# dvl-tum/e-osvos

Measured on AMD Instinct MI355X. Metric: finetune_iters_per_sec, higher is better.
Workload: dtype f32 (f16x3 split); 1 GPU; e-OSVOS-50 fine-tune iteration (BASELINE configs[1]): DeepLabV3+-ResNet50, batch 3, 480x854, BCE, per-neuron-lr SGD; one (sequence, object) per rank; batch=3, height=480, width=854, parallelism=replicas x1

## Files before the change

### e-osvos_amd/csrc/conv_kernels.hip

```cpp
#include "kernels.h"

#include <stdlib.h>
#include <string.h>

#include <vector>

namespace eosvos {

typedef float f32x16 __attribute__((ext_vector_type(16)));

#define EOSVOS_BK 32
#define EOSVOS_EB 4
#define EOSVOS_EB128 EOSVOS_EB
#define EOSVOS_OCC 2
#define MFMA32(a, b, c) __builtin_amdgcn_mfma_f32_32x32x2f32((a), (b), (c), 0, 0, 0)

__device__ __forceinline__ int xcd_remap(int bid, int nwg) {
  const int q = nwg >> 3, r = nwg & 7, xcd = bid & 7;
  return (xcd < r ? xcd * (q + 1) : r * (q + 1) + (xcd - r) * q) + (bid >> 3);
}

__device__ __forceinline__ float4 ldg4(const float* p) { return *reinterpret_cast<const float4*>(p); }
__device__ __forceinline__ float4 bufld4(__amdgpu_buffer_rsrc_t r, unsigned byte_off) {
  auto v = __builtin_amdgcn_raw_buffer_load_b128(r, byte_off, 0, 0);
// ... 764 lines not shown
    const int ks_total = p.tprefix ? p.tprefix[tile + 1] - p.tprefix[tile] : ksteps;
    unsigned long long tappack = 0x876543210ULL;
    if (!MULTI && p.tprefix) {
      const int mask = p.tmask[tile];
      tappack = 0;
      int nv = 0;
      for (int t2 = 0; t2 < T; ++t2)
        if ((mask >> t2) & 1) { tappack |= (unsigned long long)t2 << (4 * nv); ++nv; }
    }
    const int m0 = (tile / nt) * BM, n0 = (tile % nt) * BN;

    int a_sy0[APASS], a_sx0[APASS], a_img[APASS];
#pragma unroll
    for (int i = 0; i < APASS; ++i) {
      int m = m0 + a_r + i * 32;
      if (m < p.M) {
        if (p.par) m = conv_par_pixel(p.B, p.Ho, p.Wo, m);
        const int hw = p.Ho * p.Wo;
        const int b = m / hw, rem = m - b * hw;
        const int oy = rem / p.Wo, ox = rem - oy * p.Wo;
        a_sy0[i] = oy * p.mul + p.off0;
        a_sx0[i] = ox * p.mul + p.off0;
        a_img[i] = b * p.Hi * p.Wi;
      } else {
        a_sy0[i] = -(1 << 28);
        a_sx0[i] = 0;
        a_img[i] = 0;
      }
    }
    float4 ra[APASS], rb[BPASS];
    constexpr unsigned OOB = 0x80000000u;
    int a_off[APASS];
    int b_off[BPASS];
    const int wplane = p.plane_rows ? (m0 / p.plane_rows) * (int)p.w_plane : 0;
#pragma unroll
    for (int i = 0; i < BPASS; ++i) {
      if (KMAJOR) {
        const int n = n0 + b_n4 * 4;
        b_off[i] = n < p.N ? wplane + (b_kq * RPT + i) * T * p.wK + n : -1;
      } else {
        const int n = n0 + b_r + i * 32;
        b_off[i] = n < p.N ? wplane + n * T * p.wK + b_c4 * 4 : -1;
      }
    }
    int cur_tap = -1;
    int m_wrow = 0, m_ksoff = 0;
    auto load_tiles = [&](int ks) {
      const int vt = ks / chunks;
      const int c0 = (ks - vt * chunks) * BK;
      const int tap = MULTI ? vt : (p.tprefix ? (int)((tappack >> (4 * vt)) & 15) : vt);
      if (tap != cur_tap) {
        cur_tap = tap;
        int dy, dx, xoff = 0;
        if (MULTI) {
          const int id = __builtin_amdgcn_readfirstlane((int)p.taplist[(size_t)tile * 32 + vt]);
          const ConvTap d = p.taps[id];
          dy = d.dy; dx = d.dx; xoff = d.xoff; m_wrow = d.wrow; m_ksoff = d.ksoff; seg_ld = d.seg;
          if (NP == 2) { sa = pick4(seg_sa, seg_ld); sb = pick4(seg_sb, seg_ld); }
#pragma unroll
          for (int i = 0; i < BPASS; ++i) {
            const int n = n0 + b_n4 * 4;
            b_off[i] = n < p.N ? d.wbase + (b_kq * RPT + i) * d.wrow + n : -1;
          }
        } else {
          const int ky = tap / p.KW, kx = tap - ky * p.KW;
          dy = ky * p.kstep; dx = kx * p.kstep;
        }
#pragma unroll
        for (int i = 0; i < APASS; ++i) {
          const int sy = a_sy0[i] + dy, sx = a_sx0[i] + dx;
          bool ok = sy >= 0 && sx >= 0 && ((sy | sx) & (up - 1)) == 0;
          const int iy = sy >> p.upshift, ix = sx >> p.upshift;
          ok = ok && iy < p.Hi && ix < p.Wi;
          a_off[i] = ok ? (a_img[i] + iy * p.Wi + ix) * p.ldx + a_c4 * 4 + xoff : -1;
        }
      }
      const bool cok = (c0 + a_c4 * 4) < p.Kc;
      float4 ks4 = make_float4(1.f, 1.f, 1.f, 1.f);
      if (KMAJOR && p.kscale && cok) ks4 = ldg4(p.kscale + (MULTI ? m_ksoff : 0) + c0 + a_c4 * 4);
#pragma unroll
      for (int i = 0; i < APASS; ++i) {
        const unsigned off = (cok && a_off[i] >= 0) ? (unsigned)(a_off[i] + c0) * 4u : OOB;
        float4 v = bufld4(rx, off);
        if (KMAJOR) { v.x *= ks4.x; v.y *= ks4.y; v.z *= ks4.z; v.w *= ks4.w; }
        ra[i] = v;
      }
#pragma unroll
      for (int i = 0; i < BPASS; ++i) {
        unsigned off;
        if (MULTI) {
          const int k = c0 + b_kq * RPT + i;
          off = (b_off[i] >= 0 && k < p.Kc) ? (unsigned)(b_off[i] + c0 * m_wrow) * 4u : OOB;
        } else if (KMAJOR) {
          const int k = c0 + b_kq * RPT + i;
          off = (b_off[i] >= 0 && k < p.Kc) ? (unsigned)(b_off[i] + (c0 * T + tap) * p.wK) * 4u : OOB;
        } else {
          const int k = c0 + b_c4 * 4;
          off = (b_off[i] >= 0 && k < p.Kc) ? (unsigned)(b_off[i] + tap * p.wK + c0) * 4u : OOB;
        }
        rb[i] = bufld4(rw, off);
      }
    };
    auto store_tiles = [&]() {
#pragma unroll
      for (int i = 0; i < APASS; ++i) {
        uint2 pc[NP];
        xs_split4<NP>(ra[i].x, ra[i].y, ra[i].z, ra[i].w, sa, pc);
#pragma unroll
        for (int q = 0; q < NP; ++q) *reinterpret_cast<uint2*>(As + (q * BM + a_r + i * 32) * X6_ROWB + a_c4 * 8) = pc[q];
      }
      if (!KMAJOR) {
#pragma unroll
        for (int i = 0; i < BPASS; ++i) {
          uint2 pc[NP];
          xs_split4<NP>(rb[i].x, rb[i].y, rb[i].z, rb[i].w, sb, pc);
#pragma unroll
          for (int q = 0; q < NP; ++q) *reinterpret_cast<uint2*>(Bs + (q * BN + b_r + i * 32) * X6_ROWB + b_c4 * 8) = pc[q];
        }
      } else if (RPT == 4) {
#pragma unroll
        for (int j = 0; j < 4; ++j) {
          uint2 pc[NP];
          xs_split4<NP>(f4c(rb[0], j), f4c(rb[1], j), f4c(rb[RPT == 4 ? 2 : 0], j), f4c(rb[RPT == 4 ? 3 : 0], j), sb, pc);
#pragma unroll
          for (int q = 0; q < NP; ++q) *reinterpret_cast<uint2*>(Bs + (q * BN + j * NQ + b_n4) * X6_ROWB + b_kq * 8) = pc[q];
        }
      } else {
#pragma unroll
        for (int j = 0; j < 4; ++j) {
          unsigned pc[NP];
          xs_split2<NP>(f4c(rb[0], j), f4c(rb[1], j), sb, pc);
#pragma unroll
          for (int q = 0; q < NP; ++q) *reinterpret_cast<unsigned*>(Bs + (q * BN + j * NQ + b_n4) * X6_ROWB + b_kq * 4) = pc[q];
        }
      }
    };

    constexpr int TM = 4;
    f32x4 acc[TM][TN];
#pragma unroll
    for (int i = 0; i < TM; ++i)
#pragma unroll
      for (int j = 0; j < TN; ++j)
#pragma unroll
        for (int e = 0; e < 4; ++e) acc[i][j][e] = 0.f;

    load_tiles(ks_begin);
    scales_late();
    __syncthreads();
    store_tiles();
    __syncthreads();
    if (MULTI) seg_acc = seg_ld;

    for (int ks = ks_begin; ks < ks_end; ++ks) {
      const bool more = (ks + 1) < ks_end;
      if (more) load_tiles(ks + 1);
      __builtin_amdgcn_s_setprio(1);
      x6_mma_step<TM, TN, ((BN == 128 && NP == 3) ? 2 : TM), NP>(As, Bs, BM, BN, wm * 64, wn * (BN / 2), fr, fq, acc);
      __builtin_amdgcn_s_setprio(0);
      __syncthreads();
      if (more) store_tiles();
      if (MULTI && NP == 2 && more && seg_ld != seg_acc) {
        const float f = pick4(seg_inv, seg_acc) / pick4(seg_inv, seg_ld);
#pragma unroll
        for (int i = 0; i < TM; ++i)
#pragma unroll
          for (int j = 0; j < TN; ++j)
#pragma unroll
            for (int e = 0; e < 4; ++e) acc[i][j][e] *= f;
        seg_acc = seg_ld;
      }
      __syncthreads();
    }
    if (MULTI && NP == 2) inv_ab = pick4(seg_inv, seg_acc);

    float* Cs = reinterpret_cast<float*>(smem);
    const bool full = p.splitk == 0 && ks_begin == 0 && ks_end == ks_total;
    constexpr int CF4 = BN / 4, CROWS = 256 / CF4;
    const int c_c4 = tid % CF4, c_r = tid / CF4;
    const int n = n0 + c_c4 * 4;
    float4 sc = make_float4(1.f, 1.f, 1.f, 1.f), bi = make_float4(0.f, 0.f, 0.f, 0.f);
    if (full && n < p.N) {
      if (p.scale) sc = ldg4(p.scale + n);
      if (p.bias) bi = ldg4(p.bias + n);
    }
    const bool use_mask8 = p.mask8 && n >= p.mask_c0;
    const bool write_m8 = p.mask8_out && p.relu;
    const float y2s = (NP == 2 && p.y2) ? *p.y2_sc : 0.f;
    {
#pragma unroll
      for (int tm = 0; tm < TM; ++tm)
#pragma unroll
        for (int tn = 0; tn < TN; ++tn) {
          const int Rb = wn * (BN / 2) + tn * 16 + fr;
          const int ncol = KMAJOR ? x6_row_chan(Rb, BN) : Rb;
#pragma unroll
          for (int e = 0; e < 4; ++e) Cs[(wm * 64 + tm * 16 + 4 * fq + e) * LDC + ncol] = NP == 2 ? acc[tm][tn][e] * inv_ab : acc[tm][tn][e];
        }
      __syncthreads();
      if (full) {
        if (n < p.N) {
          constexpr int NIT = BM / CROWS, EB = BN == 128 ? EOSVOS_EB128 : EOSVOS_EB;
          const float* const adp = p.res ? p.res : (p.accum ? p.y : nullptr);
          const int adld = p.res ? p.ldres : p.ldy;
          const bool both = p.res && p.accum;
#pragma unroll
          for (int it0 = 0; it0 < NIT; it0 += EB) {
            size_t md[EB];
            bool ok[EB];
            float4 ad[EB];
            unsigned mk8[EB];
#pragma unroll
            for (int j = 0; j < EB; ++j) {
              const int m = m0 + c_r + (it0 + j) * CROWS;
              ok[j] = m < p.M;
              md[j] = dst_pixel(p, ok[j] ? m : p.M - 1);
            }
            if (adp) {
#pragma unroll
              for (int j = 0; j < EB; ++j) ad[j] = ldg4(adp + md[j] * adld + n);
            }
            if (use_mask8) {
#pragma unroll
              for (int j = 0; j < EB; ++j) mk8[j] = p.mask8[md[j] * p.ldm8 + (n >> 2)];
            }
#pragma unroll
            for (int j = 0; j < EB; ++j) {
              float4 v = *reinterpret_cast<const float4*>(Cs + (c_r + (it0 + j) * CROWS) * LDC + c_c4 * 4);
              if (p.scale) { v.x *= sc.x; v.y *= sc.y; v.z *= sc.z; v.w *= sc.w; }
              if (p.bias) { v.x += bi.x; v.y += bi.y; v.z += bi.z; v.w += bi.w; }
              if (adp) { v.x += ad[j].x; v.y += ad[j].y; v.z += ad[j].z; v.w += ad[j].w; }
              if (both) { const float4 a2 = ldg4(p.y + md[j] * p.ldy + n); v.x += a2.x; v.y += a2.y; v.z += a2.z; v.w += a2.w; }
              if (p.relu) { v.x = fmaxf(v.x, 0.f); v.y = fmaxf(v.y, 0.f); v.z = fmaxf(v.z, 0.f); v.w = fmaxf(v.w, 0.f); }
              if (use_mask8) relu_mask8(v, mk8[j]);
              if (ok[j]) {
                *reinterpret_cast<float4*>(p.y + md[j] * p.ldy + n) = v;
                if (write_m8) p.mask8_out[md[j] * p.ldm8_out + (n >> 2)] = relu_bits(v);
                if (NP == 2 && p.y2) pair_store4(p.y2, md[j], p.ldy, n, v, y2s);
                if (NP == 2) ymax = amax_f4(ymax, v);
              }
            }
          }
        }
      } else {
        float* slab = p.ws + ((size_t)bid * 2 + (u == u_begin ? 0 : 1)) * (BM * BN);
#pragma unroll 4
        for (int lr = c_r; lr < BM; lr += CROWS)
          *reinterpret_cast<float4*>(slab + lr * BN + c_c4 * 4) = *reinterpret_cast<const float4*>(Cs + lr * LDC + c_c4 * 4);
      }
    }
    if (!dp) u += ks_end - ks_begin;
  }
  if (NP == 2 && p.amax_y) amax_block_commit(ymax, p.amax_y);
}

template <int BN, bool KMAJOR>
__global__ __launch_bounds__(256, 2) void conv_x6_kernel(const ConvArgs p) {
  __shared__ __attribute__((aligned(16))) unsigned char smem[conv_xs_smem<BN, 3>()];
  conv_xs_body<BN, KMAJOR, 3>(p, smem);
}
#define EOSVOS_H3_OCC64 2
template <int BN, bool KMAJOR>
__global__ __launch_bounds__(256, BN == 64 ? EOSVOS_H3_OCC64 : 2) void conv_h3_kernel(const ConvArgs p) {
  __shared__ __attribute__((aligned(16))) unsigned char smem[conv_xs_smem<BN, 2>()];
  conv_xs_body<BN, KMAJOR, 2>(p, smem);
}
__global__ __launch_bounds__(256, 2) void conv_h3_multi_kernel(const ConvArgs p) {
  __shared__ __attribute__((aligned(16))) unsigned char smem[conv_xs_smem<128, 2>()];
  conv_xs_body<128, true, 2, true>(p, smem);
}
__global__ __launch_bounds__(256, 2) void conv_x6_multi_kernel(const ConvArgs p) {
  __shared__ __attribute__((aligned(16))) unsigned char smem[conv_xs_smem<128, 3>()];
  conv_xs_body<128, true, 3, true>(p, smem);
}

__device__ __forceinline__ void amax_block_commit8(unsigned m, unsigned* slot) {
  __shared__ unsigned wmax8[8];
#pragma unroll
  for (int o = 32; o > 0; o >>= 1) {
    const unsigned t = (unsigned)__shfl_xor((int)m, o);
    m = m > t ? m : t;
  }
  if ((threadIdx.x & 63) == 0) wmax8[threadIdx.x >> 6] = m;
  __syncthreads();
  if (threadIdx.x == 0) {
    unsigned q = 0;
#pragma unroll
    for (int i = 0; i < 8; ++i) q = q > wmax8[i] ? q : wmax8[i];
    if (q) atomicMax(slot + (size_t)((blockIdx.x + blockIdx.y) & (AMAX_SUB - 1)) * AMAX_ROW, q);
  }
}
__device__ __forceinline__ void s1_split8(const float4& lo, const float4& hi, float s, uint4& h0, uint4& h1) {
  unsigned a[4], b[4];
  h3_split_pair(lo.x, lo.y, s, a[0], b[0]);
  h3_split_pair(lo.z, lo.w, s, a[1], b[1]);
  h3_split_pair(hi.x, hi.y, s, a[2], b[2]);
  h3_split_pair(hi.z, hi.w, s, a[3], b[3]);
  h0 = make_uint4(a[0], a[1], a[2], a[3]);
  h1 = make_uint4(b[0], b[1], b[2], b[3]);
}
constexpr int frag_pitch(int row_bytes) { return row_bytes % 64 == 32 ? row_bytes : row_bytes + (96 - row_bytes % 64) % 64; }
#define EOSVOS_STREAM3X3_D 6
#define EOSVOS_STREAM_OCC 1
template <int K, int NC>
__global__ __launch_bounds__(512, (K <= 128 ? EOSVOS_STREAM_OCC : 1)) void conv1x1_stream_kernel(const ConvArgs p) {
  constexpr int WAVES = 8;
  constexpr int KS = (K + 31) / 32;
  constexpr int PITCH = frag_pitch(K * 2);
  constexpr int NF = NC / 16;
  constexpr int FHM = (K >= 256 || EOSVOS_STREAM_OCC > 1) ? 4 : 8;
  constexpr int FH = NF < FHM ? NF : FHM;
  constexpr bool KOUT = K >= 304;
  constexpr bool KTAIL = (K % 32) != 0;
  extern __shared__ __attribute__((aligned(16))) unsigned char s1_smem[];
  const int tid = threadIdx.x, lane = tid & 63, wave = tid >> 6;
  int n0 = blockIdx.y * NC;
  long rbase = 0, rend = p.M;
  int sbeg = blockIdx.x * WAVES + wave, sstride = gridDim.x * WAVES;
  const float* wsrc = p.w;
  if (p.plane_rows) {
    const int ranges = p.N / NC, chunks = p.row_chunks;
    const int i = blockIdx.x, xcd = i & 7, j = i >> 3;
    const int g = (j / ranges) * 8 + xcd;
    if (g >= p.nplanes * chunks) return;
    const int plane = g / chunks, chunk = g % chunks;
    const long per = (((long)p.plane_rows + chunks - 1) / chunks + 15) / 16 * 16;
    n0 = (j % ranges) * NC;
    rbase = (long)plane * p.plane_rows + chunk * per;
    rend = rbase + per;
    if (rend > (long)(plane + 1) * p.plane_rows) rend = (long)(plane + 1) * p.plane_rows;
    sbeg = wave; sstride = WAVES;
    wsrc = p.w + (size_t)plane * p.w_plane;
  }
  float* const s_sc = reinterpret_cast<float*>(s1_smem + 2 * NC * PITCH);
  float* const s_bi = s_sc + NC;
  float* const s_ks = s_bi + NC;
  static_assert(NC <= WAVES * 64 && K <= WAVES * 64, "one factor per thread");
  const float f_sc = (p.scale && tid < NC) ? p.scale[n0 + tid] : 1.f;
  const float f_bi = (p.bias && tid < NC) ? p.bias[n0 + tid] : 0.f;
  const float f_ks = (p.kscale && tid < K) ? p.kscale[tid] : 1.f;
  const unsigned ax = amax_issue(p.amax_x), aks = amax_issue(p.kmajor ? p.amax_ks : nullptr), aw = amax_issue(p.amax_w);
  float sx = 1.f, sw = 1.f, inv = 1.f;
  auto scales = [&]() {
    if (tid < NC) { s_sc[tid] = f_sc; s_bi[tid] = f_bi; }
    if (tid < KS * 32) s_ks[tid] = f_ks;
    float ix, iw;
    sx = h3_scale_bits(ax, p.kmajor && p.amax_ks, aks, ix);
    sw = h3_scale_bits(aw, false, 0u, iw);
    inv = ix * iw;
  };
  {
    constexpr int GR = NC * (K / 8), IT = (GR + WAVES * 64 - 1) / (WAVES * 64);
    if (!p.kmajor) {
      float4 raw[IT][2];
#pragma unroll
      for (int it = 0; it < IT; ++it) {
        const int i = tid + it * WAVES * 64;
        const int r = (i < GR ? i : 0) / (K / 8), c8 = i % (K / 8);
        const float* src = wsrc + (size_t)(n0 + r) * p.wK + c8 * 8;
        raw[it][0] = ldg4(src);
        raw[it][1] = ldg4(src + 4);
      }
      scales();
#pragma unroll
      for (int it = 0; it < IT; ++it) {
        const int i = tid + it * WAVES * 64;
        if (i < GR) {
          const int r = i / (K / 8), c8 = i % (K / 8);
          uint4 h0, h1;
          s1_split8(raw[it][0], raw[it][1], sw, h0, h1);
          *reinterpret_cast<uint4*>(s1_smem + r * PITCH + c8 * 16) = h0;
          *reinterpret_cast<uint4*>(s1_smem + NC * PITCH + r * PITCH + c8 * 16) = h1;
        }
      }
    } else {
      float raw[IT][8];
#pragma unroll
      for (int it = 0; it < IT; ++it) {
        const int i = tid + it * WAVES * 64;
        const int c8 = (i < GR ? i : 0) / NC, r = i % NC;
        const float* src = wsrc + (size_t)(c8 * 8) * p.wK + n0 + r;
#pragma unroll
        for (int j = 0; j < 8; ++j) raw[it][j] = src[(size_t)j * p.wK];
      }
      scales();
#pragma unroll
      for (int it = 0; it < IT; ++it) {
        const int i = tid + it * WAVES * 64;
        if (i < GR) {
          const int c8 = i / NC, r = i % NC;
          uint4 h0, h1;
          s1_split8(make_float4(raw[it][0], raw[it][1], raw[it][2], raw[it][3]), make_float4(raw[it][4], raw[it][5], raw[it][6], raw[it][7]), sw, h0, h1);
          *reinterpret_cast<uint4*>(s1_smem + r * PITCH + c8 * 16) = h0;
          *reinterpret_cast<uint4*>(s1_smem + NC * PITCH + r * PITCH + c8 * 16) = h1;
        }
      }
    }
  }
  __syncthreads();
  const int fr = lane & 15, fq = lane >> 4;
  const int nstrips = (int)((rend - rbase + 15) / 16);
  const int gw = sbeg, gstride = sstride;
  const float* const adp = p.res ? p.res : (p.accum ? p.y : nullptr);
  const int adld = p.res ? p.ldres : p.ldy;
  const bool both = p.res && p.accum;
  float4 xr[KS][2];
  auto load_x = [&](int strip) {
    const long m = rbase + (long)strip * 16 + fr;
    const float* q = p.x + (size_t)(m < rend ? m : rend - 1) * p.ldx + fq * 8;
#pragma unroll
    for (int ks = 0; ks < KS; ++ks) {
      if (!KTAIL || ks * 32 + fq * 8 < K) {
        xr[ks][0] = ldg4(q + ks * 32);
        xr[ks][1] = ldg4(q + ks * 32 + 4);
      } else {
        xr[ks][0] = xr[ks][1] = make_float4(0.f, 0.f, 0.f, 0.f);
      }
    }
  };
  unsigned ymax = 0;
  int strip = gw;
  auto load_ad = [&](int st, float4 (&ad)[FH], unsigned (&mk)[FH], int half) {
    const long m = rbase + (long)st * 16 + fr;
    const size_t r = (size_t)(m < rend ? m : rend - 1);
    if (adp) {
#pragma unroll
      for (int f = 0; f < FH; ++f) ad[f] = ldg4(adp + r * adld + n0 + (half + f) * 16 + 4 * fq);
    }
    if (p.mask8) {
#pragma unroll
      for (int f = 0; f < FH; ++f) mk[f] = p.mask8[r * p.ldm8 + ((n0 + (half + f) * 16) >> 2) + fq];
    }
  };
  if (strip < nstrips) load_x(strip);
  auto finish = [&](const f32x4& a4, int f16, const float4& adv, unsigned mkv, size_t row, bool ok) {
    const int n = n0 + f16 * 16 + 4 * fq;
    float4 v = make_float4(a4[0] * inv, a4[1] * inv, a4[2] * inv, a4[3] * inv);
    if (p.scale) { const float4 s4 = *reinterpret_cast<const float4*>(s_sc + (n - n0)); v.x *= s4.x; v.y *= s4.y; v.z *= s4.z; v.w *= s4.w; }
    if (p.bias) { const float4 b4 = *reinterpret_cast<const float4*>(s_bi + (n - n0)); v.x += b4.x; v.y += b4.y; v.z += b4.z; v.w += b4.w; }
    if (adp) { v.x += adv.x; v.y += adv.y; v.z += adv.z; v.w += adv.w; }
    if (both) { const float4 a2 = ldg4(p.y + row * p.ldy + n); v.x += a2.x; v.y += a2.y; v.z += a2.z; v.w += a2.w; }
    if (p.relu) { v.x = fmaxf(v.x, 0.f); v.y = fmaxf(v.y, 0.f); v.z = fmaxf(v.z, 0.f); v.w = fmaxf(v.w, 0.f); }
    if (p.mask8 && n >= p.mask_c0) relu_mask8(v, mkv);
    if (ok) {
      *reinterpret_cast<float4*>(p.y + row * p.ldy + n) = v;
      if (p.mask8_out && p.relu) p.mask8_out[row * p.ldm8_out + (n >> 2)] = relu_bits(v);
      ymax = amax_f4(ymax, v);
    }
  };
  if constexpr (KOUT) {
    for (; strip < nstrips; strip += gstride) {
      const int nxt = strip + gstride;
      const bool more = nxt < nstrips;
      const long mn = rbase + (long)nxt * 16 + fr;
      const float* qn = p.x + (size_t)(mn < rend ? mn : rend - 1) * p.ldx + fq * 8;
      const long m = rbase + (long)strip * 16 + fr;
      const bool ok = m < rend;
      const size_t row = (size_t)(ok ? m : rend - 1);
      f32x4 acc[NF];
#pragma unroll
      for (int f = 0; f < NF; ++f) acc[f] = f32x4{0.f, 0.f, 0.f, 0.f};
#pragma unroll
      for (int ks = 0; ks < KS; ++ks) {
        float4 a = xr[ks][0], b = xr[ks][1];
        if (more && (!KTAIL || ks * 32 + fq * 8 < K)) {
          xr[ks][0] = ldg4(qn + ks * 32);
          xr[ks][1] = ldg4(qn + ks * 32 + 4);
        }
        if (p.kscale) {
          const float4 k0 = *reinterpret_cast<const float4*>(s_ks + ks * 32 + fq * 8), k1 = *reinterpret_cast<const float4*>(s_ks + ks * 32 + fq * 8 + 4);
          a.x *= k0.x; a.y *= k0.y; a.z *= k0.z; a.w *= k0.w;
          b.x *= k1.x; b.y *= k1.y; b.z *= k1.z; b.w *= k1.w;
        }
        uint4 x0, x1;
        s1_split8(a, b, sx, x0, x1);
        const int koffs = (!KTAIL || ks * 32 + fq * 8 < K) ? ks * 64 + fq * 16 : 0;
#pragma unroll
        for (int h0 = 0; h0 < NF; h0 += FH) {
          uint4 w0[FH], w1[FH];
#pragma unroll
          for (int f = 0; f < FH; ++f) {
            const unsigned char* wp = s1_smem + ((h0 + f) * 16 + fr) * PITCH + koffs;
            w0[f] = *reinterpret_cast<const uint4*>(wp);
            w1[f] = *reinterpret_cast<const uint4*>(wp + NC * PITCH);
          }
#pragma unroll
          for (int f = 0; f < FH; ++f) acc[h0 + f] = MFMA_F16(__builtin_bit_cast(f16x8, w1[f]), __builtin_bit_cast(f16x8, x0), acc[h0 + f]);
#pragma unroll
          for (int f = 0; f < FH; ++f) acc[h0 + f] = MFMA_F16(__builtin_bit_cast(f16x8, w0[f]), __builtin_bit_cast(f16x8, x1), acc[h0 + f]);
#pragma unroll
          for (int f = 0; f < FH; ++f) acc[h0 + f] = MFMA_F16(__builtin_bit_cast(f16x8, w0[f]), __builtin_bit_cast(f16x8, x0), acc[h0 + f]);
          __builtin_amdgcn_sched_barrier(0);
        }
      }
#pragma unroll 1
      for (int h0 = 0; h0 < NF; h0 += FH) {
        float4 ad[FH];
        unsigned mk[FH];
        load_ad(strip, ad, mk, h0);
#pragma unroll
        for (int f = 0; f < FH; ++f) finish(acc[h0 + f], h0 + f, ad[f], mk[f], row, ok);
      }
    }
  } else
  for (; strip < nstrips; strip += gstride) {
    uint4 x0[KS], x1[KS];
#pragma unroll
    for (int ks = 0; ks < KS; ++ks) {
      if (p.kscale) {
        const float4 k0 = *reinterpret_cast<const float4*>(s_ks + ks * 32 + fq * 8), k1 = *reinterpret_cast<const float4*>(s_ks + ks * 32 + fq * 8 + 4);
        xr[ks][0].x *= k0.x; xr[ks][0].y *= k0.y; xr[ks][0].z *= k0.z; xr[ks][0].w *= k0.w;
        xr[ks][1].x *= k1.x; xr[ks][1].y *= k1.y; xr[ks][1].z *= k1.z; xr[ks][1].w *= k1.w;
      }
      s1_split8(xr[ks][0], xr[ks][1], sx, x0[ks], x1[ks]);
    }
    float4 ad[FH];
    unsigned mk[FH];
    const int nxt = strip + gstride;
    if (nxt < nstrips) load_x(nxt);
    const long m = rbase + (long)strip * 16 + fr;
    const bool ok = m < rend;
    const size_t row = (size_t)(ok ? m : rend - 1);
#pragma unroll 1
    for (int half = 0; half < NF; half += FH) {
      load_ad(strip, ad, mk, half);
      f32x4 acc[FH];
#pragma unroll
      for (int f = 0; f < FH; ++f) {
        acc[f] = f32x4{0.f, 0.f, 0.f, 0.f};
#pragma unroll
        for (int ks = 0; ks < KS; ++ks) {
          const unsigned char* wp = s1_smem + ((half + f) * 16 + fr) * PITCH + ks * 64 + fq * 16;
          const uint4 w0 = *reinterpret_cast<const uint4*>(wp);
          const uint4 w1 = *reinterpret_cast<const uint4*>(wp + NC * PITCH);
          acc[f] = MFMA_F16(__builtin_bit_cast(f16x8, w1), __builtin_bit_cast(f16x8, x0[ks]), acc[f]);
          acc[f] = MFMA_F16(__builtin_bit_cast(f16x8, w0), __builtin_bit_cast(f16x8, x1[ks]), acc[f]);
          acc[f] = MFMA_F16(__builtin_bit_cast(f16x8, w0), __builtin_bit_cast(f16x8, x0[ks]), acc[f]);
        }
        __builtin_amdgcn_sched_barrier(0);
      }
#pragma unroll
      for (int f = 0; f < FH; ++f) {
        finish(acc[f], half + f, ad[f], mk[f], row, ok);
        __builtin_amdgcn_sched_barrier(0);
      }
    }
  }
  if (p.amax_y) amax_block_commit8(ymax, p.amax_y);
}
template <int KC, int NC, int D>
__global__ __launch_bounds__(512, 1) void conv3x3_stream_kernel(const ConvArgs p) {
  constexpr int WAVES = 8, T = 9;
  constexpr int K = T * KC, KS = K / 32, KPT = KC / 32;
  constexpr int PITCH = frag_pitch(K * 2);
  constexpr int NF = NC / 16;
  static_assert(KS % D == 0 && NF <= 4, "ring depth must divide the K steps; every fragment's accumulator stays live");
  extern __shared__ __attribute__((aligned(16))) unsigned char s3_smem[];
  const int tid = threadIdx.x, lane = tid & 63, wave = tid >> 6;
  float* const s_sc = reinterpret_cast<float*>(s3_smem + 2 * NC * PITCH);
  float* const s_bi = s_sc + NC;
  float* const s_ks = s_bi + NC;
  constexpr int GR = NC * (K / 8), IT = (GR + WAVES * 64 - 1) / (WAVES * 64);
  static_assert(NC <= WAVES * 64 && KC <= WAVES * 64, "one factor per thread");
  const float f_sc = (p.scale && tid < NC) ? p.scale[tid] : 1.f;
  const float f_bi = (p.bias && tid < NC) ? p.bias[tid] : 0.f;
  const float f_ks = (p.kscale && tid < KC) ? p.kscale[tid] : 1.f;
  const unsigned ax = amax_issue(p.amax_x), aks = amax_issue(p.kmajor ? p.amax_ks : nullptr), aw = amax_issue(p.amax_w);
  float sx = 1.f, sw = 1.f, inv = 1.f;
  auto scales = [&]() {
    if (tid < NC) { s_sc[tid] = f_sc; s_bi[tid] = f_bi; }
    if (tid < KC) s_ks[tid] = f_ks;
    float ix, iw;
    sx = h3_scale_bits(ax, p.kmajor && p.amax_ks, aks, ix);
    sw = h3_scale_bits(aw, false, 0u, iw);
    inv = ix * iw;
  };
  if (!p.kmajor) {
    float4 raw[IT][2];
#pragma unroll
    for (int it = 0; it < IT; ++it) {
      const int i = tid + it * WAVES * 64;
      const int r = i / (K / 8), c8 = i % (K / 8);
      const float* src = p.w + (size_t)(i < GR ? r : 0) * T * p.wK + c8 * 8;
      raw[it][0] = ldg4(src);
      raw[it][1] = ldg4(src + 4);
    }
    scales();
#pragma unroll
    for (int it = 0; it < IT; ++it) {
      const int i = tid + it * WAVES * 64;
      if (i < GR) {
        const int r = i / (K / 8), c8 = i % (K / 8);
        uint4 h0, h1;
        s1_split8(raw[it][0], raw[it][1], sw, h0, h1);
        *reinterpret_cast<uint4*>(s3_smem + r * PITCH + c8 * 16) = h0;
        *reinterpret_cast<uint4*>(s3_smem + NC * PITCH + r * PITCH + c8 * 16) = h1;
      }
    }
  } else {
    float raw[IT][8];
#pragma unroll
    for (int it = 0; it < IT; ++it) {
      const int i = tid + it * WAVES * 64;
      const int c8 = (i < GR ? i : 0) / NC, r = i % NC;
      const int tap = (c8 * 8) / KC, c0 = (c8 * 8) % KC;
      const float* src = p.w + ((size_t)c0 * T + tap) * p.wK + r;
      const size_t st = (size_t)T * p.wK;
#pragma unroll
      for (int j = 0; j < 8; ++j) raw[it][j] = src[j * st];
    }
    scales();
#pragma unroll
    for (int it = 0; it < IT; ++it) {
      const int i = tid + it * WAVES * 64;
      if (i < GR) {
        const int c8 = i / NC, r = i % NC;
        uint4 h0, h1;
        s1_split8(make_float4(raw[it][0], raw[it][1], raw[it][2], raw[it][3]), make_float4(raw[it][4], raw[it][5], raw[it][6], raw[it][7]), sw, h0, h1);
        *reinterpret_cast<uint4*>(s3_smem + r * PITCH + c8 * 16) = h0;
        *reinterpret_cast<uint4*>(s3_smem + NC * PITCH + r * PITCH + c8 * 16) = h1;
      }
    }
  }
  __syncthreads();
  const int fr = lane & 15, fq = lane >> 4;
  const int nstrips = (p.M + 15) / 16;
  const int gstride = gridDim.x * WAVES;
  const float* const adp = p.res ? p.res : (p.accum ? p.y : nullptr);
  const int adld = p.res ? p.ldres : p.ldy;
  const bool both = p.res && p.accum;
  const int hw = p.Ho * p.Wo;
  struct Pix { long base, centre; unsigned ok; };
  auto pix_of = [&](int strip) {
    int m = strip * 16 + fr;
    m = m < p.M ? m : p.M - 1;
    const int b = m / hw, rem = m - b * hw;
    const int oy = rem / p.Wo, ox = rem - oy * p.Wo;
    Pix q;
    q.base = (((long)b * p.Hi + oy + p.off0) * p.Wi + ox + p.off0) * p.ldx + fq * 8;
    q.centre = (((long)b * p.Hi + oy) * p.Wi + ox) * p.ldx + fq * 8;
    q.ok = 0;
#pragma unroll
    for (int k3 = 0; k3 < 3; ++k3) {
      const int sy = oy + p.off0 + k3 * p.kstep, sx2 = ox + p.off0 + k3 * p.kstep;
      if (sy >= 0 && sy < p.Hi) q.ok |= 1u << k3;
      if (sx2 >= 0 && sx2 < p.Wi) q.ok |= 8u << k3;
    }
    return q;
  };
  float4 ring[D][2];
  auto tap_ok = [&](const Pix& q, int ks) {
    const int tap = ks / KPT, ky = tap / 3, kx = tap % 3;
    return ((q.ok >> ky) & (q.ok >> (3 + kx)) & 1u) != 0;
  };
  auto load_k = [&](const Pix& q, int ks, float4 (&dst)[2]) {
    const int tap = ks / KPT, kin = ks % KPT, ky = tap / 3, kx = tap % 3;
    const long off = tap_ok(q, ks) ? q.base + ((long)ky * p.kstep * p.Wi + kx * p.kstep) * p.ldx : q.centre;
    const float* src = p.x + off + kin * 32;
    dst[0] = ldg4(src);
    dst[1] = ldg4(src + 4);
  };
  unsigned ymax = 0;
  int strip = blockIdx.x * WAVES + wave;
  Pix cur = pix_of(strip < nstrips ? strip : 0);
  if (strip < nstrips) {
#pragma unroll
    for (int d = 0; d < D; ++d) load_k(cur, d, ring[d]);
  }
  for (; strip < nstrips; strip += gstride) {
    const int nxt = strip + gstride;
    const bool more = nxt < nstrips;
    const Pix nx = pix_of(more ? nxt : strip);
    const int m = strip * 16 + fr;
    const bool ok = m < p.M;
    const size_t row = (size_t)(ok ? m : p.M - 1);
    f32x4 acc[NF];
#pragma unroll
    for (int f = 0; f < NF; ++f) acc[f] = f32x4{0.f, 0.f, 0.f, 0.f};
    const bool border = __any(cur.ok != 0x3fu);
#pragma unroll
    for (int ks = 0; ks < KS; ++ks) {
      float4& a = ring[ks % D][0];
      float4& b = ring[ks % D][1];
      if (border && !tap_ok(cur, ks)) a = b = make_float4(0.f, 0.f, 0.f, 0.f);
      if (p.kscale) {
        const int kin = ks % KPT;
        const float4 k0 = *reinterpret_cast<const float4*>(s_ks + kin * 32 + fq * 8), k1 = *reinterpret_cast<const float4*>(s_ks + kin * 32 + fq * 8 + 4);
        a.x *= k0.x; a.y *= k0.y; a.z *= k0.z; a.w *= k0.w;
        b.x *= k1.x; b.y *= k1.y; b.z *= k1.z; b.w *= k1.w;
      }
      uint4 x0, x1;
      s1_split8(a, b, sx, x0, x1);
      if (ks + D < KS) load_k(cur, ks + D, ring[ks % D]);
      else load_k(nx, ks + D - KS, ring[ks % D]);
      uint4 w0[NF], w1[NF];
#pragma unroll
      for (int f = 0; f < NF; ++f) {
        const unsigned char* wp = s3_smem + (f * 16 + fr) * PITCH + ks * 64 + fq * 16;
        w0[f] = *reinterpret_cast<const uint4*>(wp);
        w1[f] = *reinterpret_cast<const uint4*>(wp + NC * PITCH);
      }
#pragma unroll
      for (int f = 0; f < NF; ++f) acc[f] = MFMA_F16(__builtin_bit_cast(f16x8, w1[f]), __builtin_bit_cast(f16x8, x0), acc[f]);
#pragma unroll
      for (int f = 0; f < NF; ++f) acc[f] = MFMA_F16(__builtin_bit_cast(f16x8, w0[f]), __builtin_bit_cast(f16x8, x1), acc[f]);
#pragma unroll
      for (int f = 0; f < NF; ++f) acc[f] = MFMA_F16(__builtin_bit_cast(f16x8, w0[f]), __builtin_bit_cast(f16x8, x0), acc[f]);
      __builtin_amdgcn_sched_barrier(0);
    }
#pragma unroll
    for (int f = 0; f < NF; ++f) {
      const int n = f * 16 + 4 * fq;
      float4 v = make_float4(acc[f][0] * inv, acc[f][1] * inv, acc[f][2] * inv, acc[f][3] * inv);
      if (p.scale) { const float4 s4 = *reinterpret_cast<const float4*>(s_sc + n); v.x *= s4.x; v.y *= s4.y; v.z *= s4.z; v.w *= s4.w; }
      if (p.bias) { const float4 b4 = *reinterpret_cast<const float4*>(s_bi + n); v.x += b4.x; v.y += b4.y; v.z += b4.z; v.w += b4.w; }
      if (adp) { const float4 a4 = ldg4(adp + row * adld + n); v.x += a4.x; v.y += a4.y; v.z += a4.z; v.w += a4.w; }
      if (both) { const float4 a2 = ldg4(p.y + row * p.ldy + n); v.x += a2.x; v.y += a2.y; v.z += a2.z; v.w += a2.w; }
      if (p.relu) { v.x = fmaxf(v.x, 0.f); v.y = fmaxf(v.y, 0.f); v.z = fmaxf(v.z, 0.f); v.w = fmaxf(v.w, 0.f); }
      if (p.mask8 && n >= p.mask_c0) relu_mask8(v, p.mask8[row * p.ldm8 + (n >> 2)]);
      if (ok) {
        *reinterpret_cast<float4*>(p.y + row * p.ldy + n) = v;
        if (p.mask8_out && p.relu) p.mask8_out[row * p.ldm8_out + (n >> 2)] = relu_bits(v);
        ymax = amax_f4(ymax, v);
      }
    }
    cur = nx;
  }
  if (p.amax_y) amax_block_commit8(ymax, p.amax_y);
}
static bool stream3x3_ok(const ConvArgs& a) {
  constexpr int min_m = 16384;
  if (conv_mfma_mode() != 2 || a.nseg > 0 || a.plane_rows || a.KH != 3 || a.KW != 3 || a.upshift || a.dst_up || a.par ||
      a.tprefix || a.mul != 1 || a.M < min_m)
    return false;
  if (a.Kc != 64 || a.N != 64 || a.wK != 64) return false;
  if ((a.mask_c0 & 15) || (a.ldx & 3) || (a.ldy & 3)) return false;
  if (a.Hi != a.Ho || a.Wi != a.Wo) return false;
  if (!(a.kstep == 1 || a.kstep == -1) || a.off0 != -a.kstep) return false;
  return true;
}
static void launch_stream3x3(const ConvArgs& a, hipStream_t s) {
  constexpr int KC = 64, NC = 64, D = EOSVOS_STREAM3X3_D;
  constexpr int lds = 2 * NC * frag_pitch(9 * KC * 2) + (2 * NC + KC) * 4;
  static bool attr = false;
  if (!attr) { (void)hipFuncSetAttribute((const void*)conv3x3_stream_kernel<KC, NC, D>, hipFuncAttributeMaxDynamicSharedMemorySize, lds); attr = true; }
  hipLaunchKernelGGL((conv3x3_stream_kernel<KC, NC, D>), dim3(256), dim3(512), lds, s, a);
}
static int stream1x1_nc(const ConvArgs& a) {
  const int min_m = a.B == 1 && !a.plane_rows ? 1024 : 16384;
  if (conv_mfma_mode() != 2 || a.nseg > 0 || a.KH != 1 || a.KW != 1 || a.upshift || a.dst_up || a.par ||
      a.tprefix || a.mul != 1 || a.off0 != 0 || a.M < min_m)
    return 0;
  if (a.plane_rows) {
    if (a.mask8 || a.res || a.accum || a.scale || a.bias || a.relu || a.kscale || a.amax_y) return 0;
    if ((a.ldx & 3) || (a.ldy & 3) || (a.plane_rows & 15)) return 0;
    if (a.Kc != 256 && !(a.Kc == 304 && !a.kmajor)) return 0;
    if (a.N % 128 == 0) return 128;
    if (a.N % 64 == 0) return 64;
    if (a.N == 48 && a.Kc == 256) return 48;
    return 0;
  }
  if (a.Kc != 64 && a.Kc != 128 && a.Kc != 256 && a.Kc != 512) return 0;
  if ((a.mask_c0 & 15) || (a.ldx & 3) || (a.ldy & 3) || (a.N & 15)) return 0;
  if (a.Hi != a.Ho || a.Wi != a.Wo) return 0;
  if (a.Kc == 512) return a.N % 64 == 0 && a.N <= 128 ? 64 : 0;
  if (a.N % 128 == 0) return 128;
  if (a.N == 64) return 64;
  if (a.N == 48 && a.Kc == 256) return 48;
  return 0;
}
template <int K, int NC>
static void launch_stream1x1(ConvArgs& a, hipStream_t s) {
  constexpr int lds = 2 * NC * frag_pitch(K * 2) + (2 * NC + (K + 31) / 32 * 32) * 4;
  static bool attr = false;
  if (!attr) { (void)hipFuncSetAttribute((const void*)conv1x1_stream_kernel<K, NC>, hipFuncAttributeMaxDynamicSharedMemorySize, lds); attr = true; }
  if (a.plane_rows) {
    constexpr int target = 216;
    const int ranges = a.N / NC;
    int chunks = (target + a.nplanes * ranges - 1) / (a.nplanes * ranges);
    const int max_chunks = a.plane_rows / 128 > 0 ? a.plane_rows / 128 : 1;
    chunks = chunks < 1 ? 1 : (chunks > max_chunks ? max_chunks : chunks);
    a.row_chunks = chunks;
    const int groups8 = (a.nplanes * chunks + 7) / 8 * 8;
    hipLaunchKernelGGL((conv1x1_stream_kernel<K, NC>), dim3(groups8 * ranges), dim3(512), lds, s, a);
    return;
  }
  constexpr int total = 256 * (K <= 128 ? EOSVOS_STREAM_OCC : 1);
  const int ranges = a.N / NC;
  const int wgs = total / ranges > 0 ? total / ranges : 1;
  hipLaunchKernelGGL((conv1x1_stream_kernel<K, NC>), dim3(wgs, ranges), dim3(512), lds, s, a);
}


#define STEM_SLOTS 24
#define STEM_PITCH (STEM_SLOTS * 16 + 32)
__global__ __launch_bounds__(512) void stem_fwd_h3_kernel(const float* __restrict__ xpad, const float* __restrict__ w,
                                                          const float* __restrict__ a, const float* __restrict__ bb,
                                                          float* __restrict__ y, int B, int H, int W, int Ho, int Wo,
                                                          const unsigned* __restrict__ amax_x) {
  __shared__ __attribute__((aligned(16))) unsigned char sw_[2 * 64 * STEM_PITCH];
  __shared__ float s_a[64], s_b[64];
  __shared__ unsigned s_red[8];
  const int tid = threadIdx.x, lane = tid & 63, wave = tid >> 6;
  float wv[3][8];
  unsigned wm = 0;
#pragma unroll
  for (int q = 0; q < 3; ++q) {
    const int i = tid + q * 512, r = i / STEM_SLOTS, sl = i % STEM_SLOTS;
    const int ky = sl / 3, part = sl % 3;
#pragma unroll
    for (int t = 0; t < 8; ++t) {
      const int j = part * 8 + t;
      const float v = (sl < 21 && j < 21) ? w[r * 147 + ky * 21 + j] : 0.f;
      wv[q][t] = v;
      const unsigned b = amax_f1(v);
      wm = wm > b ? wm : b;
    }
  }
#pragma unroll
  for (int o = 32; o > 0; o >>= 1) {
    const unsigned t = (unsigned)__shfl_xor((int)wm, o);
    wm = wm > t ? wm : t;
  }
  if (lane == 0) s_red[wave] = wm;
  if (tid < 64) { s_a[tid] = a ? a[tid] : 1.f; s_b[tid] = bb ? bb[tid] : 0.f; }
  __syncthreads();
#pragma unroll
  for (int i = 0; i < 8; ++i) wm = wm > s_red[i] ? wm : s_red[i];
  float sw, iw;
  {
    const int e = (int)((wm >> 23) & 0xffu);
    int f = 268 - e;
    f = f < 1 ? 1 : (f > 254 ? 254 : f);
    iw = __uint_as_float((unsigned)(254 - f) << 23);
    sw = __uint_as_float((unsigned)f << 23);
  }
#pragma unroll
  for (int q = 0; q < 3; ++q) {
    const int i = tid + q * 512, r = i / STEM_SLOTS, sl = i % STEM_SLOTS;
    uint4 h0, h1;
    s1_split8(make_float4(wv[q][0], wv[q][1], wv[q][2], wv[q][3]), make_float4(wv[q][4], wv[q][5], wv[q][6], wv[q][7]), sw, h0, h1);
    *reinterpret_cast<uint4*>(sw_ + r * STEM_PITCH + sl * 16) = h0;
    *reinterpret_cast<uint4*>(sw_ + 64 * STEM_PITCH + r * STEM_PITCH + sl * 16) = h1;
  }
  float ix;
  const float sx = h3_scale(amax_x, nullptr, ix);
  const float inv = ix * iw;
  __syncthreads();
  const int fr = lane & 15, fq = lane >> 4;
  const int Wp = W + 6, Hp = H + 6;
  const long P = (long)B * Ho * Wo;
  const long nstrips = (P + 15) / 16;
  int koff[6];
  int ktail = 0;
#pragma unroll
  for (int ks = 0; ks < 6; ++ks) {
    const int sl = ks * 4 + fq;
    koff[ks] = sl < 21 ? (sl / 3) * Wp * 3 + (sl % 3) * 8 : -1;
    if (sl < 21 && sl % 3 == 2) ktail |= 1 << ks;
  }
  float2 xr[6][4];
  auto load_x = [&](long strip) {
    long pp = strip * 16 + fr;
    pp = pp < P ? pp : P - 1;
    const int ox = (int)(pp % Wo), oy = (int)((pp / Wo) % Ho), b = (int)(pp / ((long)Wo * Ho));
    const float* base = xpad + (((long)b * Hp + oy * 2) * Wp + ox * 2) * 3;
#pragma unroll
    for (int ks = 0; ks < 6; ++ks) {
      if (koff[ks] >= 0) {
        const float2* q = reinterpret_cast<const float2*>(base + koff[ks]);
#pragma unroll
        for (int t = 0; t < 4; ++t) xr[ks][t] = q[t];
        if (ktail & (1 << ks)) { xr[ks][2].y = 0.f; xr[ks][3] = make_float2(0.f, 0.f); }
      } else {
#pragma unroll
        for (int t = 0; t < 4; ++t) xr[ks][t] = make_float2(0.f, 0.f);
      }
    }
  };
  const long gw = (long)blockIdx.x * 8 + wave, gstride = (long)gridDim.x * 8;
  long strip = gw;
  if (strip < nstrips) load_x(strip);
  for (; strip < nstrips; strip += gstride) {
    uint4 x0[6], x1[6];
#pragma unroll
    for (int ks = 0; ks < 6; ++ks)
      s1_split8(make_float4(xr[ks][0].x, xr[ks][0].y, xr[ks][1].x, xr[ks][1].y), make_float4(xr[ks][2].x, xr[ks][2].y, xr[ks][3].x, xr[ks][3].y),
                sx, x0[ks], x1[ks]);
    if (strip + gstride < nstrips) load_x(strip + gstride);
    const long pp = strip * 16 + fr;
    const bool ok = pp < P;
#pragma unroll
    for (int f = 0; f < 4; ++f) {
      f32x4 acc = {0.f, 0.f, 0.f, 0.f};
#pragma unroll
      for (int ks = 0; ks < 6; ++ks) {
        const unsigned char* wp = sw_ + (f * 16 + fr) * STEM_PITCH + ks * 64 + fq * 16;
        const uint4 w0 = *reinterpret_cast<const uint4*>(wp);
        const uint4 w1 = *reinterpret_cast<const uint4*>(wp + 64 * STEM_PITCH);
        acc = MFMA_F16(__builtin_bit_cast(f16x8, w1), __builtin_bit_cast(f16x8, x0[ks]), acc);
        acc = MFMA_F16(__builtin_bit_cast(f16x8, w0), __builtin_bit_cast(f16x8, x1[ks]), acc);
        acc = MFMA_F16(__builtin_bit_cast(f16x8, w0), __builtin_bit_cast(f16x8, x0[ks]), acc);
      }
      const int n = f * 16 + 4 * fq;
      float4 v = make_float4(acc[0] * inv, acc[1] * inv, acc[2] * inv, acc[3] * inv);
      if (a) {
        const float4 a4 = *reinterpret_cast<const float4*>(s_a + n), b4 = *reinterpret_cast<const float4*>(s_b + n);
        v.x = fmaxf(v.x * a4.x + b4.x, 0.f); v.y = fmaxf(v.y * a4.y + b4.y, 0.f);
        v.z = fmaxf(v.z * a4.z + b4.z, 0.f); v.w = fmaxf(v.w * a4.w + b4.w, 0.f);
      }
      if (ok) *reinterpret_cast<float4*>(y + pp * 64 + n) = v;
      __builtin_amdgcn_sched_barrier(0);
    }
  }
}
void launch_stem_fwd_h3(const float* xpad, const float* w, const float* a, const float* b, float* y, int B, int H, int W, int Ho,
                        int Wo, const unsigned* amax_x, hipStream_t s) {
  hipLaunchKernelGGL(stem_fwd_h3_kernel, dim3(256), dim3(512), 0, s, xpad, w, a, b, y, B, H, W, Ho, Wo, amax_x);
}

__global__ __launch_bounds__(256, 2) void stem_wgrad_h3_kernel(const float* __restrict__ xpad, const float* __restrict__ g,
                                                               float* __restrict__ ws, int B, int H, int W, int Ho, int Wo,
                                                               int chunks, const unsigned* __restrict__ amax_g,
                                                               const unsigned* __restrict__ amax_x) {
  constexpr int KR = 160;
  __shared__ __attribute__((aligned(16))) unsigned char As[2 * 64 * X6_ROWB];
  __shared__ __attribute__((aligned(16))) unsigned char Bs[2 * KR * X6_ROWB];
  const long P = (long)B * Ho * Wo;
  const long per = ((P + chunks - 1) / chunks + 31) / 32 * 32;
  const long p0 = (long)blockIdx.x * per;
  long p1 = p0 + per;
  if (p1 > P) p1 = P;
  const int tid = threadIdx.x, lane = tid & 63, wave = __builtin_amdgcn_readfirstlane(tid >> 6);
  const int fr = lane & 15, fq = lane >> 4;
  const int Wp = W + 6, Hp = H + 6;
  const int k = tid;
  const int koff = k < 147 ? (k / 21) * Wp * 3 + (k % 21) : 0;
  const int a_cg = tid & 15, a_pg = tid >> 4;
  float ig, ix;
  const unsigned ag_w = amax_issue(amax_g), ax_w = amax_issue(amax_x);
  const float sg = h3_scale_bits(ag_w, false, 0u, ig), sx = h3_scale_bits(ax_w, false, 0u, ix);
  f32x4 acc[10];
#pragma unroll
  for (int j = 0; j < 10; ++j) acc[j] = f32x4{0.f, 0.f, 0.f, 0.f};
  for (int i = tid; i < 2 * (KR - 147) * (X6_ROWB / 4); i += 256) {
    const int pc = i / ((KR - 147) * (X6_ROWB / 4)), rem = i % ((KR - 147) * (X6_ROWB / 4));
    *reinterpret_cast<unsigned*>(Bs + (pc * KR + 147) * X6_ROWB + rem * 4) = 0u;
  }
  const int nsteps = p1 > p0 ? (int)((p1 - p0 + 31) / 32) : 0;
  float4 ra[2];
  float rb[32];
  auto load_step = [&](int st) {
    const long ps = p0 + (long)st * 32;
#pragma unroll
    for (int i = 0; i < 2; ++i) {
      const long px = ps + a_pg * 2 + i;
      ra[i] = px < p1 ? ldg4(g + px * 64 + a_cg * 4) : make_float4(0.f, 0.f, 0.f, 0.f);
    }
    if (k < 147) {
      int ox = (int)(ps % Wo), oy = (int)((ps / Wo) % Ho), b = (int)(ps / ((long)Wo * Ho));
      long base = (((long)b * Hp + oy * 2) * Wp + ox * 2) * 3 + koff;
#pragma unroll
      for (int i = 0; i < 32; ++i) {
        rb[i] = (ps + i) < p1 ? xpad[base] : 0.f;
        base += 6;
        if (++ox == Wo) {
          ox = 0;
          base += (long)(2 * Wp - 2 * Wo) * 3;
          if (++oy == Ho) { oy = 0; base += (long)(Hp - 2 * Ho) * Wp * 3; }
        }
      }
    }
  };
  auto store_step = [&]() {
#pragma unroll
    for (int j = 0; j < 4; ++j) {
      unsigned pc[2];
      xs_split2<2>(f4c(ra[0], j), f4c(ra[1], j), sg, pc);
      *reinterpret_cast<unsigned*>(As + (a_cg * 4 + j) * X6_ROWB + a_pg * 4) = pc[0];
      *reinterpret_cast<unsigned*>(As + (64 + a_cg * 4 + j) * X6_ROWB + a_pg * 4) = pc[1];
    }
    if (k < 147) {
#pragma unroll
      for (int q = 0; q < 4; ++q) {
        uint4 h0, h1;
        s1_split8(make_float4(rb[8 * q], rb[8 * q + 1], rb[8 * q + 2], rb[8 * q + 3]),
                  make_float4(rb[8 * q + 4], rb[8 * q + 5], rb[8 * q + 6], rb[8 * q + 7]), sx, h0, h1);
        *reinterpret_cast<uint4*>(Bs + k * X6_ROWB + q * 16) = h0;
        *reinterpret_cast<uint4*>(Bs + (KR + k) * X6_ROWB + q * 16) = h1;
      }
    }
  };
  if (nsteps > 0) load_step(0);
  __syncthreads();
  if (nsteps > 0) store_step();
  __syncthreads();
  for (int st = 0; st < nsteps; ++st) {
    const bool more = st + 1 < nsteps;
    if (more) load_step(st + 1);
    const uint4 a0 = *reinterpret_cast<const uint4*>(As + (wave * 16 + fr) * X6_ROWB + fq * 16);
    const uint4 a1 = *reinterpret_cast<const uint4*>(As + (64 + wave * 16 + fr) * X6_ROWB + fq * 16);
#pragma unroll
    for (int j = 0; j < 10; ++j) {
      const uint4 b0 = *reinterpret_cast<const uint4*>(Bs + (j * 16 + fr) * X6_ROWB + fq * 16);
      const uint4 b1 = *reinterpret_cast<const uint4*>(Bs + (KR + j * 16 + fr) * X6_ROWB + fq * 16);
      acc[j] = MFMA_F16(__builtin_bit_cast(f16x8, a1), __builtin_bit_cast(f16x8, b0), acc[j]);
      acc[j] = MFMA_F16(__builtin_bit_cast(f16x8, a0), __builtin_bit_cast(f16x8, b1), acc[j]);
      acc[j] = MFMA_F16(__builtin_bit_cast(f16x8, a0), __builtin_bit_cast(f16x8, b0), acc[j]);
    }
    __syncthreads();
    if (more) store_step();
    __syncthreads();
  }
  const float inv = ig * ix;
  float* out = ws + (long)blockIdx.x * (64 * 147);
#pragma unroll
  for (int j = 0; j < 10; ++j) {
    const int kk = j * 16 + fr;
    if (kk < 147) {
#pragma unroll
      for (int e = 0; e < 4; ++e) out[(wave * 16 + 4 * fq + e) * 147 + kk] = acc[j][e] * inv;
    }
  }
}
void launch_stem_wgrad_h3(const float* xpad, const float* g, float* ws, int B, int H, int W, int Ho, int Wo, int chunks,
                          const unsigned* amax_g, const unsigned* amax_x, hipStream_t s) {
  hipLaunchKernelGGL(stem_wgrad_h3_kernel, dim3(chunks), dim3(256), 0, s, xpad, g, ws, B, H, W, Ho, Wo, chunks, amax_g, amax_x);
}


template <int BMO, int BNI, int NP> constexpr int wgrad_xs_smem() { return xs_max(NP * (BMO + BNI) * X6_ROWB, BMO * (BNI + 4) * 4); }
template <int BMO, int BNI, int NP = 3>
__device__ __forceinline__ void wgrad_x6_body(const WgradArgs& p, const int bid, unsigned char* smem) {
  constexpr int BKP = 32;
  constexpr int A_BYTES = NP * BMO * X6_ROWB;
  constexpr int LDC = BNI + 4;
  unsigned char* const As = smem;
  unsigned char* const Bs = smem + A_BYTES;

  const int tid = threadIdx.x, lane = tid & 63, wave = tid >> 6;
  const int wm = wave >> 1, wn = wave & 1;
  const int fr = lane & 15, fq = lane >> 4;

  const int T = p.KH * p.KW;
  const int ct = (p.Cout + BMO - 1) / BMO, it = (p.Cin + BNI - 1) / BNI;
  const int tiles = ct * it * T;
  const int z = bid / tiles;
  int tile = bid - z * tiles;
  const int tap = tile % T; tile /= T;
  const int co0 = (tile / it) * BMO, ci0 = (tile % it) * BNI;
  const int ky = tap / p.KW, kx = tap - ky * p.KW;

  const int dyk = ky * p.dil - p.pad, dxk = kx * p.dil - p.pad;
  auto cdiv = [](int a, int b) { return a >= 0 ? (a + b - 1) / b : -((-a) / b); };
  auto fdiv = [](int a, int b) { return a >= 0 ? a / b : -((-a + b - 1) / b); };
  int oy_lo = cdiv(-dyk, p.stride), oy_hi = fdiv(p.Hi - 1 - dyk, p.stride);
  int ox_lo = cdiv(-dxk, p.stride), ox_hi = fdiv(p.Wi - 1 - dxk, p.stride);
  if (oy_lo < 0) oy_lo = 0;
  if (ox_lo < 0) ox_lo = 0;
  if (oy_hi > p.Ho - 1) oy_hi = p.Ho - 1;
  if (ox_hi > p.Wo - 1) ox_hi = p.Wo - 1;
  const int hv = oy_hi - oy_lo + 1 > 0 ? oy_hi - oy_lo + 1 : 0;
  const int wv = ox_hi - ox_lo + 1 > 0 ? ox_hi - ox_lo + 1 : 0;
  const int P = p.B * hv * wv;
  const int steps = (P + BKP - 1) / BKP;
  const int st_begin = (int)(((long)steps * z) / p.splits);
  const int st_end = (int)(((long)steps * (z + 1)) / p.splits);

  constexpr int ANQ = BMO / 4, ARPT = BMO / 32, BNQ = BNI / 4, BRPT = BNI / 32;
  const int a_c4 = ARPT == 4 ? x6_kmaj_c4_128(tid) : x6_kmaj_c4_64(tid), a_kq = ARPT == 4 ? x6_kmaj_kq_128(tid) : x6_kmaj_kq_64(tid);
  const int b_c4 = BRPT == 4 ? x6_kmaj_c4_128(tid) : x6_kmaj_c4_64(tid), b_kq = BRPT == 4 ? x6_kmaj_kq_128(tid) : x6_kmaj_kq_64(tid);
  const bool a_cok = (co0 + a_c4 * 4) < p.Cout;
  const bool b_cok = (ci0 + b_c4 * 4) < p.Cin;
  float4 ra[ARPT], rb[BRPT];
  constexpr unsigned OOB = 0x80000000u;
  const __amdgpu_buffer_rsrc_t rg = make_rsrc(p.g + tap * p.g_tap_stride, (long)p.B * p.Ho * p.Wo * p.ldg * 4);
// ... 736 lines not shown
```

Measured before the change: 113.7 finetune_iters/s.

## Coalesce activation loads in 1x1 stream conv via per-wave LDS staging

For the K=256/NC=64 and K=128/NC=128 instantiations of the streaming 1x1 conv, activation rows are now loaded so that consecutive lanes read contiguous 16-byte pieces of a row chunk, instead of each lane reading strided fragment positions. The loaded values are split into f16 hi/lo pairs, written to a per-wave LDS tile, and read back in MFMA fragment layout, with wave-level barriers in between. The aim is better global-load coalescing for the activation stream. In exchange it adds LDS traffic, extra dynamic LDS per block and wave syncs inside the strip loop.

```diff
diff --git a/e-osvos_amd/csrc/conv_kernels.hip b/e-osvos_amd/csrc/conv_kernels.hip
--- a/e-osvos_amd/csrc/conv_kernels.hip
+++ b/e-osvos_amd/csrc/conv_kernels.hip
@@ -1090,6 +1090,7 @@
 constexpr int frag_pitch(int row_bytes) { return row_bytes % 64 == 32 ? row_bytes : row_bytes + (96 - row_bytes % 64) % 64; }
 #define EOSVOS_STREAM3X3_D 6
 #define EOSVOS_STREAM_OCC 1
+constexpr int stream1x1_stage_xk(int K, int NC) { return (K == 256 && NC == 64) || (K == 128 && NC == 128) ? 128 : 0; }
 template <int K, int NC>
 __global__ __launch_bounds__(512, (K <= 128 ? EOSVOS_STREAM_OCC : 1)) void conv1x1_stream_kernel(const ConvArgs p) {
   constexpr int WAVES = 8;
@@ -1098,6 +1099,11 @@
   constexpr int NF = NC / 16;
   constexpr int FHM = (K >= 256 || EOSVOS_STREAM_OCC > 1) ? 4 : 8;
   constexpr int FH = NF < FHM ? NF : FHM;
+  constexpr int XK = stream1x1_stage_xk(K, NC);
+  constexpr int XKD = XK ? XK : 64;
+  constexpr int XP = frag_pitch(XKD * 2);
+  constexpr int XLPR = XKD / 4, XRPI = 64 / XLPR, XIPC = 16 / XRPI, XCH = K / XKD;
+  static_assert(XK == 0 || (K < 304 && K % XK == 0), "whole chunks, no K tail, the plain loop form");
   constexpr bool KOUT = K >= 304;
   constexpr bool KTAIL = (K % 32) != 0;
   extern __shared__ __attribute__((aligned(16))) unsigned char s1_smem[];
@@ -1193,7 +1199,22 @@
   const int adld = p.res ? p.ldres : p.ldy;
   const bool both = p.res && p.accum;
   float4 xr[KS][2];
+  unsigned char* const tile_x = s1_smem + 2 * NC * PITCH + (2 * NC + KS * 32) * 4 + wave * (2 * 16 * XP);
+  const int xrl = lane / XLPR, xq = lane % XLPR;
+  auto wave_sync = [&]() {
+    __builtin_amdgcn_fence(__ATOMIC_RELEASE, "wavefront");
+    __builtin_amdgcn_wave_barrier();
+    __builtin_amdgcn_fence(__ATOMIC_ACQUIRE, "wavefront");
+  };
   auto load_x = [&](int strip) {
+    if constexpr (XK != 0) {
+#pragma unroll
+      for (int i = 0; i < KS * 2; ++i) {
+        const long m = rbase + (long)strip * 16 + (i % XIPC) * XRPI + xrl;
+        xr[i / 2][i % 2] = ldg4(p.x + (size_t)(m < rend ? m : rend - 1) * p.ldx + (i / XIPC) * XK + 4 * xq);
+      }
+      return;
+    }
     const long m = rbase + (long)strip * 16 + fr;
     const float* q = p.x + (size_t)(m < rend ? m : rend - 1) * p.ldx + fq * 8;
 #pragma unroll
@@ -1293,6 +1314,33 @@
   } else
   for (; strip < nstrips; strip += gstride) {
     uint4 x0[KS], x1[KS];
+    if constexpr (XK != 0) {
+#pragma unroll
+      for (int c = 0; c < XCH; ++c) {
+#pragma unroll
+        for (int i = 0; i < XIPC; ++i) {
+          float4 v = xr[(c * XIPC + i) / 2][(c * XIPC + i) % 2];
+          if (p.kscale) {
+            const float4 k4 = *reinterpret_cast<const float4*>(s_ks + c * XK + 4 * xq);
+            v.x *= k4.x; v.y *= k4.y; v.z *= k4.z; v.w *= k4.w;
+          }
+          unsigned a0, b0, a1, b1;
+          h3_split_pair(v.x, v.y, sx, a0, b0);
+          h3_split_pair(v.z, v.w, sx, a1, b1);
+          unsigned char* const dst = tile_x + (i * XRPI + xrl) * XP + xq * 8;
+          *reinterpret_cast<uint2*>(dst) = make_uint2(a0, a1);
+          *reinterpret_cast<uint2*>(dst + 16 * XP) = make_uint2(b0, b1);
+        }
+        wave_sync();
+#pragma unroll
+        for (int kl = 0; kl < XK / 32; ++kl) {
+          const unsigned char* const src = tile_x + fr * XP + kl * 64 + fq * 16;
+          x0[c * (XK / 32) + kl] = *reinterpret_cast<const uint4*>(src);
+          x1[c * (XK / 32) + kl] = *reinterpret_cast<const uint4*>(src + 16 * XP);
+        }
+        wave_sync();
+      }
+    } else {
 #pragma unroll
     for (int ks = 0; ks < KS; ++ks) {
       if (p.kscale) {
@@ -1301,6 +1349,7 @@
         xr[ks][1].x *= k1.x; xr[ks][1].y *= k1.y; xr[ks][1].z *= k1.z; xr[ks][1].w *= k1.w;
       }
       s1_split8(xr[ks][0], xr[ks][1], sx, x0[ks], x1[ks]);
+    }
     }
     float4 ad[FH];
     unsigned mk[FH];
@@ -1559,7 +1608,9 @@
 }
 template <int K, int NC>
 static void launch_stream1x1(ConvArgs& a, hipStream_t s) {
-  constexpr int lds = 2 * NC * frag_pitch(K * 2) + (2 * NC + (K + 31) / 32 * 32) * 4;
+  constexpr int xk = stream1x1_stage_xk(K, NC);
+  constexpr int lds = 2 * NC * frag_pitch(K * 2) + (2 * NC + (K + 31) / 32 * 32) * 4 + (xk ? 8 * 2 * 16 * frag_pitch(xk * 2) : 0);
+  static_assert(lds + 64 <= 163840, "weight image, factors and activation tiles fit the CU's LDS");
   static bool attr = false;
   if (!attr) { (void)hipFuncSetAttribute((const void*)conv1x1_stream_kernel<K, NC>, hipFuncAttributeMaxDynamicSharedMemorySize, lds); attr = true; }
   if (a.plane_rows) {
```

Result: no change. 114.0 finetune_iters/s (median of 4 runs) (+0.3%).
